# benfred/implicit

Hardware: AMD Instinct MI355X
Metric: ALS user+item updates/sec per iteration (factors=128); top-k recs/sec (higher is better)
Workload: dtype f32; 1 GPU; BASELINE configs[2]: last.fm-360K-shaped synthetic CSR, ALS CG cg_steps=3; users=358868, items=292385, nnz=17308340, factors=128, solver=cg, cg_steps=3

## Files before the change

### implicit_amd/csrc/als_cg_q.hip

```cpp
#include <type_traits>

#include "als_qtile.h"
#include "common.h"

namespace imp {

template <typename T>
void launch_team_fused(const imp_csr *C, int f, int width, int first, int count, T *X, const T *Y, const float *A0, int cg_steps,
                       const char *name);
template <typename T>
void launch_group_fused(const imp_csr *C, int f, int first, int count, T *X, const T *Y, const float *A0, int cg_steps, const char *name);
template <typename ST>
void launch_team_tile64(const imp_csr *C, int f, int width, int first, int count, ST *X, const ST *Y, const float *A0, int cg_steps,
                        const char *name);

template <int F, typename T> static void run_classes_q(const imp_csr *C, T *X, const T *Y, const float *A0, int cg_steps) {
  const int32_t *b = C->bin_start;
  constexpr bool kHalf = std::is_same<T, __half>::value;
  auto team = [&](int width32, int lo, int hi, const char *name) {
    if constexpr (kHalf) launch_team_tile64<T>(C, F, width32 / 2, lo, hi - lo, X, Y, A0, cg_steps, name);
    else launch_team_fused<T>(C, F, width32, lo, hi - lo, X, Y, A0, cg_steps, name);
  };
  team(16, b[1], b[2], "als_cg_team16_rows");
  team(8, b[2], b[3], "als_cg_team8_rows");
  team(4, b[3], b[4], "als_cg_team4_rows");
  team(2, b[4], b[5], "als_cg_team2_rows");
  if constexpr (F == 64) launch_team_fused<T>(C, F, 1, b[5], b[7] - b[5], X, Y, A0, cg_steps, "als_cg_short_rows");
  else launch_group_fused<T>(C, F, b[5], b[7] - b[5], X, Y, A0, cg_steps, "als_cg_short_rows");
}

template <typename T> void least_squares_cg_q(const imp_csr *C, T *X, const T *Y, const float *A0, int f, int cg_steps) {
  if (f == 128) run_classes_q<128, T>(C, X, Y, A0, cg_steps);
  else if (f == 64) run_classes_q<64, T>(C, X, Y, A0, cg_steps);
  else throw std::invalid_argument("least_squares_cg_q: f must be 64 or 128");
}
template void least_squares_cg_q<float>(const imp_csr *, float *, const float *, const float *, int, int);
template void least_squares_cg_q<__half>(const imp_csr *, __half *, const __half *, const float *, int, int);

}
```

### implicit_amd/csrc/als_cg_qf.hip

```cpp
#include <type_traits>

#include "als_qf_common.h"
#include "common.h"

namespace imp {

template <typename ST> struct Tile32 {
  typedef f32x2 elem;
  static constexpr int T = 32;
  static constexpr bool ROLL = std::is_same<ST, float>::value;
  static __device__ __forceinline__ void fetch(const int32_t *indices, const float *data, int lane, int k0, int end, int &col, float &c) {
    fetch_entries(indices, data, lane, k0, end, col, c);
  }
  template <int H> static __device__ __forceinline__ void gather(elem (&yq)[H], const ST *p) {
#pragma unroll
    for (int h = 0; h < H; h += 2) {
      const float4 v = load4(p + 32 * h);
      yq[h] = f32x2{v.x, v.y}, yq[h + 1] = f32x2{v.z, v.w};
    }
  }
  template <int H> static __device__ __forceinline__ float dot(const elem (&yq)[H], const f32x2 (&ve)[H]) {
    f32x2 s = yq[0] * ve[0];
#pragma unroll
    for (int h = 1; h < H; ++h) s = __builtin_elementwise_fma(yq[h], ve[h], s);
    return s.x + s.y;
  }
  template <int H> static __device__ __forceinline__ void axpy(const elem (&yq)[H], float w, f32x2 (&ae)[H]) {
    const f32x2 w2 = {w, w};
#pragma unroll
    for (int h = 0; h < H; ++h) ae[h] = __builtin_elementwise_fma(w2, yq[h], ae[h]);
  }
};

template <int F, int WPR, int BLOCK, typename ST>
__global__ __launch_bounds__(BLOCK, F == 64 ? 8 : 4) void als_cg_qfteam_kernel(const int32_t *__restrict__ order, int first, int count,
                                                                 const int32_t *__restrict__ indptr,
                                                                 const int32_t *__restrict__ indices,
                                                                 const float *__restrict__ data, ST *__restrict__ X,
                                                                 const ST *__restrict__ Y, const float *__restrict__ A0,
                                                                 int cg_steps) {
  team_rows<Tile32<ST>, F, WPR, BLOCK>(order, first, count, indptr, indices, data, X, Y, A0, cg_steps);
}

template <int F, int WPR, int BLOCK, typename T>
static void launch_qfteam(const imp_csr *C, int first, int count, T *X, const T *Y, const float *A0, int cg_steps,
                          const char *name) {
  if (count <= 0) return;
  constexpr int WAVES = BLOCK / 64, TEAMS = WAVES / WPR;
  size_t lds = team_lds_bytes<F, WPR, BLOCK, Tile32<T>::T>();
  auto kern = als_cg_qfteam_kernel<F, WPR, BLOCK, T>;
  IMP_CHECK_HIP(hipFuncSetAttribute(reinterpret_cast<const void *>(kern), hipFuncAttributeMaxDynamicSharedMemorySize, (int)lds));
  int per_cu = (int)std::max<size_t>(1, std::min<size_t>(2048 / BLOCK, (160 * 1024) / lds));
  constexpr int kBaseOversub = WPR <= 4 ? 4 : (WPR == 8 ? 2 : (F == 64 ? 2 : 1));
  int grid = std::min((count + TEAMS - 1) / TEAMS, ctx().num_cus * per_cu * std::max(kBaseOversub, ctx().oversub));
  IMP_PROF(name);
  kern<<<grid, BLOCK, lds, stream()>>>(C->order.data(), first, count, C->indptr.data(), C->indices.data(), C->data.data(), X, Y,
                                      A0, cg_steps);
  IMP_CHECK_HIP(hipGetLastError());
}

typedef float f32x4 __attribute__((ext_vector_type(4)));
template <int F> struct QFGroupCfg {
  static constexpr int LD = F + 8;
  static constexpr int LDB = F + 8;
  static constexpr int NT = F / 16;
  static constexpr int KH = 16 / NT;
  static constexpr int KB = (F / 16) / KH;
  static constexpr size_t lds_bytes = (size_t)3 * F * LDB * 2 + (size_t)3 * 16 * LDB * 2 +
                                      ((size_t)16 * LD + (size_t)KH * 16 * LD + 16 * 64) * sizeof(float);
};
typedef __bf16 bf16x8 __attribute__((ext_vector_type(8)));
typedef __bf16 bf16x2 __attribute__((ext_vector_type(2)));
__device__ __forceinline__ void split_bf16(float x, __bf16 &hi, __bf16 &mid, __bf16 &lo) {
  hi = (__bf16)x;
  const float r1 = x - (float)hi;
  mid = (__bf16)r1;
  lo = (__bf16)(r1 - (float)mid);
}

template <int F, bool FIRST, bool LAST, typename ST>
__device__ __forceinline__ void tile_pass(f32x2 (&y)[8][F / 32], float *cw, int cnt, const float *vrow, float (&acc)[F / 64], int lane,
                                          int cnt_nx, int &col_nx, float &c_nx, const ST *__restrict__ Y) {
  using Tile = Tile32<ST>;
  constexpr int FE = F / 16, H = FE / 2;
  if constexpr (LAST) {
    col_nx = opaque(col_nx);
    c_nx = __int_as_float(opaque(__float_as_int(c_nx)));
  }
  f32x2 ve[H], ae[H];
  const float *cwg;
  {
    const int ln = opaque(lane);
    const int g = ln >> 4, m = ln & 15;
#pragma unroll
    for (int e = 0; e < FE; e += 4) {
      const float4 t = *reinterpret_cast<const float4 *>(vrow + 16 * e + 4 * m);
      ve[e / 2] = f32x2{t.x, t.y}, ve[e / 2 + 1] = f32x2{t.z, t.w};
    }
    cwg = cw + g;
  }
#pragma unroll
  for (int h = 0; h < H; ++h) ae[h] = f32x2{0.f, 0.f};
  auto partial = [&](int q) { return Tile::template dot<H>(y[q], ve); };
  auto axpy = [&](int q, float w) { Tile::template axpy<H>(y[q], w, ae); };
  static_for<4>([&](auto Pc) {
    constexpr int P = decltype(Pc)::value;
    if (8 * P < cnt) {
      const float cm1_0 = cwg[8 * P], cm1_1 = cwg[8 * P + 4];
      float cp_0 = 0.f, cp_1 = 0.f;
      if constexpr (FIRST) cp_0 = cwg[32 + 8 * P], cp_1 = cwg[32 + 8 * P + 4];
      const float u = reduce_pair(partial(2 * P), partial(2 * P + 1));
      const float w0 = FIRST ? fmaf(-cm1_0, row_bcast_from<0>(u), cp_0) : cm1_0 * row_bcast_from<0>(u);
      const float w1 = FIRST ? fmaf(-cm1_1, row_bcast_from<8>(u), cp_1) : cm1_1 * row_bcast_from<8>(u);
      axpy(2 * P, w0);
      axpy(2 * P + 1, w1);
    }
    if constexpr (LAST) {
      if (8 * P < cnt_nx) gather_pair<Tile, F, P>(y, cw, col_nx, c_nx, cnt_nx, Y, lane);
    }
  });
  float aes[FE];
#pragma unroll
  for (int h = 0; h < H; ++h) aes[2 * h] = ae[h].x, aes[2 * h + 1] = ae[h].y;
  reduce_expanded<F>(aes, acc);
}

template <int F, typename ST>
__global__ __launch_bounds__(1024) void als_cg_qfgroup_kernel(const int32_t *__restrict__ order, int first, int count,
                                                              const int32_t *__restrict__ indptr,
                                                              const int32_t *__restrict__ indices,
                                                              const float *__restrict__ data, ST *__restrict__ X,
                                                              const ST *__restrict__ Y, const float *__restrict__ A0, int cg_steps) {
  using Cfg = QFGroupCfg<F>;
  constexpr int FC = F / 64, FE = F / 16, LD = Cfg::LD;
  constexpr bool ROLL = Tile32<ST>::ROLL;
  extern __shared__ __attribute__((aligned(16))) float smem[];
  constexpr int LDB = Cfg::LDB;
  __bf16 *A0b = reinterpret_cast<__bf16 *>(smem);
  __bf16 *Pb = A0b + (size_t)3 * F * LDB;
  float *Ps = reinterpret_cast<float *>(Pb + (size_t)3 * 16 * LDB);
  float *Outs = Ps + 16 * LD;
  float *cws = Outs + (size_t)Cfg::KH * 16 * LD;
  const int lane = threadIdx.x & 63;
  const int wave = __builtin_amdgcn_readfirstlane(threadIdx.x >> 6);
  for (int e = threadIdx.x; e < F * F; e += 1024) {
    int r = e / F, c = e - r * F;
    __bf16 h, m, l;
    split_bf16(A0[e], h, m, l);
    A0b[r * LDB + c] = h, A0b[(size_t)F * LDB + r * LDB + c] = m, A0b[(size_t)2 * F * LDB + r * LDB + c] = l;
  }
  __syncthreads();
  float *prow = Ps + (size_t)wave * LD;
  float *cw = cws + (size_t)wave * 64;
  const unsigned cf = (unsigned)QL<F>::cfactor(lane, 0);

  auto publish = [&](const float (&vec)[FC], bool valid) {
    if constexpr (FC == 2) *reinterpret_cast<float2 *>(prow + cf) = valid ? make_float2(vec[0], vec[1]) : make_float2(0.f, 0.f);
    else prow[cf] = valid ? vec[0] : 0.f;
    bf16x2 t[3];
#pragma unroll
    for (int c = 0; c < 2; ++c) {
      __bf16 h, m, l;
      split_bf16(valid ? vec[c] : 0.f, h, m, l);
      t[0][c] = h, t[1][c] = m, t[2][c] = l;
    }
#pragma unroll
    for (int k = 0; k < 3; ++k) *reinterpret_cast<bf16x2 *>(Pb + (size_t)k * 16 * LDB + (size_t)wave * LDB + cf) = t[k];
    __syncthreads();
  };
  auto product = [&]() {
    const int ti = wave % Cfg::NT, kh = wave / Cfg::NT;
    const int ln = opaque(lane);
    const int i = ln & 15, kq = ln >> 4;
    f32x4 acc = {0.f, 0.f, 0.f, 0.f};
    static_assert(Cfg::KB * 16 == 64, "three-term product: 64 k per wave");
#pragma unroll
    for (int b = 0; b < 2; ++b) {
      const int k0 = kh * 64 + 32 * b + 8 * kq;
      const __bf16 *ar = A0b + (size_t)(16 * ti + i) * LDB + k0, *pr = Pb + (size_t)i * LDB + k0;
      const bf16x8 ah = *reinterpret_cast<const bf16x8 *>(ar), am = *reinterpret_cast<const bf16x8 *>(ar + (size_t)F * LDB),
                   al = *reinterpret_cast<const bf16x8 *>(ar + (size_t)2 * F * LDB);
      const bf16x8 ph = *reinterpret_cast<const bf16x8 *>(pr), pm = *reinterpret_cast<const bf16x8 *>(pr + (size_t)16 * LDB),
                   pl = *reinterpret_cast<const bf16x8 *>(pr + (size_t)2 * 16 * LDB);
      acc = __builtin_amdgcn_mfma_f32_16x16x32_bf16(al, ph, acc, 0, 0, 0);
      acc = __builtin_amdgcn_mfma_f32_16x16x32_bf16(ah, pl, acc, 0, 0, 0);
      acc = __builtin_amdgcn_mfma_f32_16x16x32_bf16(am, pm, acc, 0, 0, 0);
      acc = __builtin_amdgcn_mfma_f32_16x16x32_bf16(am, ph, acc, 0, 0, 0);
      acc = __builtin_amdgcn_mfma_f32_16x16x32_bf16(ah, pm, acc, 0, 0, 0);
      acc = __builtin_amdgcn_mfma_f32_16x16x32_bf16(ah, ph, acc, 0, 0, 0);
    }
    *reinterpret_cast<float4 *>(Outs + (kh * 16 + i) * LD + 16 * ti + 4 * kq) = make_float4(acc[0], acc[1], acc[2], acc[3]);
  };
  auto collect = [&](float (&out)[FC]) {
#pragma unroll
    for (int c = 0; c < FC; ++c) out[c] = 0.f;
#pragma unroll
    for (int h = 0; h < Cfg::KH; ++h) {
      const float *o = Outs + (h * 16 + wave) * LD + cf;
      if constexpr (FC == 2) {
        const float2 t = *reinterpret_cast<const float2 *>(o);
        out[0] += t.x, out[1] += t.y;
      } else {
        out[0] += o[0];
      }
    }
  };
  const bool product_first = ((wave >> 2) & 1) == 0;

  const int groups = (count + 15) / 16, g_step = gridDim.x;
  auto row_id = [&](int g) { return order[first + min(g * 16 + wave, count - 1)]; };
  auto row_valid = [&](int g) { return g < groups && g * 16 + wave < count; };
  int id0 = row_id(blockIdx.x), id1 = row_id(blockIdx.x + g_step), id2 = row_id(blockIdx.x + 2 * g_step), id3 = row_id(blockIdx.x + 3 * g_step);
  int b0 = indptr[id0], e0 = indptr[id0 + 1], b1 = indptr[id1], e1 = indptr[id1 + 1], b2 = indptr[id2], e2 = indptr[id2 + 1];
  int ent_col, ent_cnt = row_valid(blockIdx.x) ? e0 - b0 : 0;
  float ent_c;
  fetch_entries(indices, data, opaque(lane), b0, max(e0, b0 + 1), ent_col, ent_c);
  bool tile_ready = false;
  int cnt = 0;
  f32x2 y[8][FE / 2];
  float x[FC];
  auto kill = [](float (&v)[FC]) {
#pragma unroll
    for (int cc = 0; cc < FC; ++cc) v[cc] = 0.f;
  };
  kill(x);
  for (int g = blockIdx.x; g < groups; g += g_step) {
    const bool valid = row_valid(g);
    ST *xrow = X + (size_t)id0 * F;
    if (!tile_ready) {
      cnt = ent_cnt;
      ent_col = opaque(ent_col);
      ent_c = __int_as_float(opaque(__float_as_int(ent_c)));
      static_for<4>([&](auto Pc) {
        constexpr int P = decltype(Pc)::value;
        if (8 * P < cnt) gather_pair<Tile32<ST>, F, P>(y, cw, ent_col, ent_c, cnt, Y, lane);
      });
      ent_cnt = row_valid(g + g_step) ? e1 - b1 : 0;
      fetch_entries(indices, data, opaque(lane), b1, max(e1, b1 + 1), ent_col, ent_c);
      load_compact<F>(xrow, opaque(lane), x);
    }
    float xc[FC], r[FC], p[FC], Ap[FC], sp[FC];
#pragma unroll
    for (int cc = 0; cc < FC; ++cc) xc[cc] = x[cc];
    publish(xc, valid);
    if (!product_first) tile_pass<F, true, false, ST>(y, cw, cnt, prow, sp, lane, 0, ent_col, ent_c, Y);
    product();
    if (product_first) tile_pass<F, true, false, ST>(y, cw, cnt, prow, sp, lane, 0, ent_col, ent_c, Y);
    __syncthreads();
    collect(Ap);
#pragma unroll
    for (int cc = 0; cc < FC; ++cc) p[cc] = r[cc] = sp[cc] - Ap[cc];
    float rsold = dot_compact<F>(r, r);
    bool active = valid && rsold >= 1e-20f;
    const bool store = active;
    for (int it = 0; it + 1 < cg_steps; ++it) {
      publish(p, active);
      if (active && !product_first) tile_pass<F, false, false, ST>(y, cw, cnt, prow, sp, lane, 0, ent_col, ent_c, Y);
      product();
      if (active && product_first) tile_pass<F, false, false, ST>(y, cw, cnt, prow, sp, lane, 0, ent_col, ent_c, Y);
      __syncthreads();
      collect(Ap);
      if (active) {
#pragma unroll
        for (int cc = 0; cc < FC; ++cc) Ap[cc] += sp[cc];
        const float alpha = rsold * __builtin_amdgcn_rcpf(dot_compact<F>(p, Ap));
#pragma unroll
        for (int cc = 0; cc < FC; ++cc) {
          xc[cc] = fmaf(alpha, p[cc], xc[cc]);
          r[cc] = fmaf(-alpha, Ap[cc], r[cc]);
        }
        const float rsnew = dot_compact<F>(r, r);
        if (rsnew < 1e-20f) {
          active = false;
        } else {
          const float beta = rsnew * __builtin_amdgcn_rcpf(rsold);
#pragma unroll
          for (int cc = 0; cc < FC; ++cc) p[cc] = fmaf(beta, p[cc], r[cc]);
          rsold = rsnew;
        }
      }
    }
    bool rolled = false;
    if (cg_steps > 0) {
      publish(p, active);
      auto last_tiles = [&]() {
        if constexpr (ROLL) tile_pass<F, false, true, ST>(y, cw, cnt, prow, sp, lane, ent_cnt, ent_col, ent_c, Y);
        else tile_pass<F, false, false, ST>(y, cw, cnt, prow, sp, lane, 0, ent_col, ent_c, Y);
      };
      if (active && !product_first) last_tiles();
      product();
      if (active && product_first) last_tiles();
      __syncthreads();
      collect(Ap);
      if (active) {
        if constexpr (ROLL) {
          cnt = ent_cnt;
          ent_cnt = row_valid(g + 2 * g_step) ? e2 - b2 : 0;
          fetch_entries(indices, data, opaque(lane), b2, max(e2, b2 + 1), ent_col, ent_c);
          load_compact<F>(X + (size_t)id1 * F, opaque(lane), x);
          rolled = true;
        } else {
          kill(x);
        }
#pragma unroll
        for (int cc = 0; cc < FC; ++cc) Ap[cc] += sp[cc];
        const float alpha = rsold * __builtin_amdgcn_rcpf(dot_compact<F>(p, Ap));
#pragma unroll
        for (int cc = 0; cc < FC; ++cc) xc[cc] = fmaf(alpha, p[cc], xc[cc]);
      } else {
        kill(x);
      }
    } else {
      kill(x);
    }
    if (store) store_compact<F>(xrow, opaque(lane), xc);
    tile_ready = rolled;
    id0 = id1, id1 = id2, id2 = id3, id3 = row_id(g + 4 * g_step);
    b0 = b1, e0 = e1, b1 = b2, e1 = e2, b2 = indptr[id2], e2 = indptr[id2 + 1];
  }
}

template <typename T>
static void launch_qfgroup(const imp_csr *C, int first, int count, T *X, const T *Y, const float *A0, int cg_steps, const char *name) {
  if (count <= 0) return;
  constexpr int F = 128;
  const size_t lds = QFGroupCfg<F>::lds_bytes;
  auto kern = als_cg_qfgroup_kernel<F, T>;
  IMP_CHECK_HIP(hipFuncSetAttribute(reinterpret_cast<const void *>(kern), hipFuncAttributeMaxDynamicSharedMemorySize, (int)lds));
  int grid = std::min((count + 15) / 16, ctx().num_cus * std::max(2, ctx().oversub));
  IMP_PROF(name);
  kern<<<grid, 1024, lds, stream()>>>(C->order.data(), first, count, C->indptr.data(), C->indices.data(), C->data.data(), X, Y, A0,
                                      cg_steps);
  IMP_CHECK_HIP(hipGetLastError());
}

template <typename T>
void launch_group_fused(const imp_csr *C, int f, int first, int count, T *X, const T *Y, const float *A0, int cg_steps, const char *name) {
  if (f == 128) launch_qfgroup<T>(C, first, count, X, Y, A0, cg_steps, name);
  else throw std::invalid_argument("launch_group_fused: f must be 128 (f = 64 short rows run on independent wavefronts)");
}
template void launch_group_fused<float>(const imp_csr *, int, int, int, float *, const float *, const float *, int, const char *);
template void launch_group_fused<__half>(const imp_csr *, int, int, int, __half *, const __half *, const float *, int, const char *);

template <typename T>
void launch_team_fused(const imp_csr *C, int f, int width, int first, int count, T *X, const T *Y, const float *A0, int cg_steps,
                       const char *name) {
  if constexpr (std::is_same<T, __half>::value) {
    if (f != 64 || width != 1) throw std::invalid_argument("launch_team_fused: float16 storage takes the f = 64 short rows only");
    launch_qfteam<64, 1, 512, T>(C, first, count, X, Y, A0, cg_steps, name);
  } else {
    auto run = [&](auto Fc) {
      constexpr int F = decltype(Fc)::value;
      switch (width) {
        case 16: launch_qfteam<F, 16, 1024, T>(C, first, count, X, Y, A0, cg_steps, name); break;
        case 8: launch_qfteam<F, 8, 512, T>(C, first, count, X, Y, A0, cg_steps, name); break;
        case 4: launch_qfteam<F, 4, 512, T>(C, first, count, X, Y, A0, cg_steps, name); break;
        case 2: launch_qfteam<F, 2, 512, T>(C, first, count, X, Y, A0, cg_steps, name); break;
        case 1:
          if constexpr (F == 64) launch_qfteam<F, 1, 512, T>(C, first, count, X, Y, A0, cg_steps, name);
          else throw std::invalid_argument("launch_team_fused: one wave per row needs f = 64");
          break;
        default: throw std::invalid_argument("launch_team_fused: team width");
      }
    };
    if (f == 128) run(idx_t<128>{});
    else if (f == 64) run(idx_t<64>{});
    else throw std::invalid_argument("launch_team_fused: f must be 64 or 128");
  }
}
template void launch_team_fused<float>(const imp_csr *, int, int, int, int, float *, const float *, const float *, int, const char *);
template void launch_team_fused<__half>(const imp_csr *, int, int, int, int, __half *, const __half *, const float *, int,
                                        const char *);

}
```

### implicit_amd/csrc/als_qf_common.h

```cpp
#ifndef IMPLICIT_AMD_CSRC_ALS_QF_COMMON_H_
#define IMPLICIT_AMD_CSRC_ALS_QF_COMMON_H_
#include <type_traits>
#include <utility>

#include "als_qtile.h"

namespace imp {

__device__ __forceinline__ int opaque(int v) {
  asm volatile("" : "+v"(v));
  return v;
}

typedef float f32x2 __attribute__((ext_vector_type(2)));

template <int I> using idx_t = std::integral_constant<int, I>;
template <int N, typename Fn, int... Is> __device__ __forceinline__ void static_for_impl(Fn &&fn, std::integer_sequence<int, Is...>) {
  (fn(idx_t<Is>{}), ...);
}
template <int N, typename Fn> __device__ __forceinline__ void static_for(Fn &&fn) {
  static_for_impl<N>(fn, std::make_integer_sequence<int, N>{});
}

template <int F, int NJ, int TICKS> struct DenseTicks {
  static constexpr int FE = F / 16, Q4 = FE / 4;
  static constexpr int EVERY = TICKS / NJ;
  static_assert(NJ >= 1 && NJ <= TICKS && TICKS % NJ == 0 && (NJ & (NJ - 1)) == 0, "steps per pass");
  float4 a[Q4];
  f32x2 vj2;
  template <int K> __device__ __forceinline__ void issue(const float *row, const float *vp) {
    if constexpr (K % EVERY == 0) {
      constexpr int s = K / EVERY;
      if constexpr (NJ == 1) vj2 = f32x2{vp[0], 0.f};
      else if constexpr (s % 2 == 0) vj2 = *reinterpret_cast<const f32x2 *>(vp + s);
#pragma unroll
      for (int e = 0; e < Q4; ++e) a[e] = *reinterpret_cast<const float4 *>(row + (size_t)s * F + 64 * e);
    }
  }
  template <int K> __device__ __forceinline__ void consume(f32x2 (&ae)[FE / 2]) {
    if constexpr (K % EVERY == 0) {
      constexpr int s = K / EVERY;
      const float vj = (s % 2 == 0) ? vj2.x : vj2.y;
      const f32x2 v2 = {vj, vj};
#pragma unroll
      for (int e = 0; e < Q4; ++e) {
        ae[2 * e] = __builtin_elementwise_fma(v2, f32x2{a[e].x, a[e].y}, ae[2 * e]);
        ae[2 * e + 1] = __builtin_elementwise_fma(v2, f32x2{a[e].z, a[e].w}, ae[2 * e + 1]);
      }
    }
  }
};

__device__ __forceinline__ float reduce_pair(float d0, float d1) {
  float u = d1 + dpp_mov<0x128>(d1);
  const float s0 = d0 + dpp_mov<0x128>(d0);
  u = __builtin_bit_cast(float, __builtin_amdgcn_update_dpp(__builtin_bit_cast(int, u), __builtin_bit_cast(int, s0), 0xE4, 0xF, 0x3,
                                                            false));
  u += dpp_mov<0x141>(u);
  u += dpp_mov<0xB1>(u);
  u += dpp_mov<0x4E>(u);
  return u;
}
template <int LANE> __device__ __forceinline__ float row_bcast_from(float v) {
  return dpp_mov<0x150 + LANE>(v);
}

enum : unsigned { kGo = 1u, kLast = 2u };

#ifndef IMP_TEAM_NAP_FIRST
#define IMP_TEAM_NAP_FIRST 6
#endif
#ifndef IMP_TEAM_NAP_NEXT
#define IMP_TEAM_NAP_NEXT 2
#endif
#ifndef IMP_TEAM_NAP_LEADER
#define IMP_TEAM_NAP_LEADER 1
#endif
#ifndef IMP_TEAM_LEADER_PRIO
#define IMP_TEAM_LEADER_PRIO 0
#endif


template <typename Tile, int F, int P, typename ST>
__device__ __forceinline__ void gather_pair(typename Tile::elem (&y)[Tile::T / 4][F / 32], float *cw, int col_reg, float c_reg, int cnt,
                                            const ST *__restrict__ Y, int lane) {
  lane = opaque(lane);
  if ((lane >> 3) == P) {
    const bool ok = lane < cnt;
    cw[lane] = ok ? fabsf(c_reg) - 1.f : 0.f;
    cw[Tile::T + lane] = ok ? fmaxf(c_reg, 0.f) : 0.f;
  }
  const int src = 4 * (lane >> 4);
#pragma unroll
  for (int q = 2 * P; q < 2 * P + 2; ++q) {
    const unsigned col = (unsigned)__builtin_amdgcn_ds_bpermute(src + 16 * q, col_reg);
    Tile::template gather<F / 32>(y[q], Y + (size_t)col * F + 4 * (lane & 15));
  }
}

template <typename Tile, int F, int NJ, bool FIRST, bool LAST, typename ST>
__device__ __forceinline__ void fused_pass(typename Tile::elem (&y)[Tile::T / 4][F / 32], float *cw, int cnt, const float *vt,
                                           int j_begin, const float *A0s, float (&acc)[F / 64], int lane, int cnt_nx, int &col_nx,
                                           float &c_nx, const ST *__restrict__ Y, const int32_t *__restrict__ indices,
                                           const float *__restrict__ data, int k0_nx2, int end_nx2) {
  constexpr int FE = F / 16, H = FE / 2, PAIRS = Tile::T / 8;
  if constexpr (LAST) {
    col_nx = opaque(col_nx);
    c_nx = __int_as_float(opaque(__float_as_int(c_nx)));
  }
  f32x2 ve[H], ae[H];
  const float *row, *vp, *cwg;
  {
    const int ln = opaque(lane);
    const int g = ln >> 4, m = ln & 15;
#pragma unroll
    for (int e = 0; e < FE; e += 4) {
      const float4 t = *reinterpret_cast<const float4 *>(vt + 16 * e + 4 * m);
      ve[e / 2] = f32x2{t.x, t.y}, ve[e / 2 + 1] = f32x2{t.z, t.w};
    }
    vp = vt + j_begin + g * NJ;
    row = A0s + (size_t)(j_begin + g * NJ) * F + 4 * m;
    cwg = cw + g;
  }
#pragma unroll
  for (int h = 0; h < H; ++h) ae[h] = f32x2{0.f, 0.f};
  DenseTicks<F, NJ, 4 * PAIRS> dt;
  auto partial = [&](int q) { return Tile::template dot<H>(y[q], ve); };
  auto axpy = [&](int q, float w) { Tile::template axpy<H>(y[q], w, ae); };
  static_for<PAIRS>([&](auto Pc) {
    constexpr int P = decltype(Pc)::value;
    if (8 * P < cnt) {
      dt.template issue<4 * P>(row, vp);
      const float cm1_0 = cwg[8 * P], cm1_1 = cwg[8 * P + 4];
      float cp_0 = 0.f, cp_1 = 0.f;
      if constexpr (FIRST) cp_0 = cwg[Tile::T + 8 * P], cp_1 = cwg[Tile::T + 8 * P + 4];
      __builtin_amdgcn_sched_barrier(0);
      const float d0 = partial(2 * P);
      __builtin_amdgcn_sched_barrier(0);
      dt.template consume<4 * P>(ae);
      dt.template issue<4 * P + 1>(row, vp);
      __builtin_amdgcn_sched_barrier(0);
      const float d1 = partial(2 * P + 1);
      const float u = reduce_pair(d0, d1);
      dt.template consume<4 * P + 1>(ae);
      const float w0 = FIRST ? fmaf(cm1_0, row_bcast_from<0>(u), -cp_0) : cm1_0 * row_bcast_from<0>(u);
      const float w1 = FIRST ? fmaf(cm1_1, row_bcast_from<8>(u), -cp_1) : cm1_1 * row_bcast_from<8>(u);
      __builtin_amdgcn_sched_barrier(0);
      dt.template issue<4 * P + 2>(row, vp);
      __builtin_amdgcn_sched_barrier(0);
      axpy(2 * P, w0);
      __builtin_amdgcn_sched_barrier(0);
      dt.template consume<4 * P + 2>(ae);
      dt.template issue<4 * P + 3>(row, vp);
      __builtin_amdgcn_sched_barrier(0);
      axpy(2 * P + 1, w1);
      __builtin_amdgcn_sched_barrier(0);
      dt.template consume<4 * P + 3>(ae);
    } else {
      asm volatile("" ::: "memory");
      static_for<4>([&](auto Kc) {
        constexpr int K = 4 * P + decltype(Kc)::value;
        dt.template issue<K>(row, vp);
        __builtin_amdgcn_sched_barrier(0);
        dt.template consume<K>(ae);
      });
    }
    if constexpr (LAST) {
      if (8 * P < cnt_nx) gather_pair<Tile, F, P>(y, cw, col_nx, c_nx, cnt_nx, Y, lane);
    }
    __builtin_amdgcn_sched_barrier(0);
  });
  float aes[FE];
#pragma unroll
  for (int h = 0; h < H; ++h) aes[2 * h] = ae[h].x, aes[2 * h + 1] = ae[h].y;
  reduce_expanded<F>(aes, acc);
  if constexpr (LAST) {
    Tile::fetch(indices, data, opaque(lane), k0_nx2, end_nx2, col_nx, c_nx);
  }
}

template <int F, int WPR, int BLOCK, int T> constexpr size_t team_lds_bytes() {
  constexpr size_t WAVES = BLOCK / 64, TEAMS = WAVES / WPR;
  return ((size_t)F * F + WAVES * F + TEAMS * F + 2 * T * WAVES + 4 * TEAMS) * sizeof(float);
}

template <typename Tile, int F, int WPR, int BLOCK, typename ST>
__device__ __forceinline__ void team_rows(const int32_t *__restrict__ order, int first, int count, const int32_t *__restrict__ indptr,
                                          const int32_t *__restrict__ indices, const float *__restrict__ data, ST *__restrict__ X,
                                          const ST *__restrict__ Y, const float *__restrict__ A0, int cg_steps) {
  constexpr int FC = F / 64, FE = F / 16, T = Tile::T, WAVES = BLOCK / 64, TEAMS = WAVES / WPR, NJ = F / WPR / 4;
  static_assert(WPR <= WAVES && (F / WPR) % 4 == 0, "team width");
  extern __shared__ __attribute__((aligned(16))) float smem[];
  float *A0s = smem;
  float *parts = A0s + (size_t)F * F;
  float *vts = parts + (size_t)WAVES * F;
  float *cws = vts + (size_t)TEAMS * F;
  unsigned *ctl = reinterpret_cast<unsigned *>(cws + (size_t)WAVES * 2 * T);
  const int lane = threadIdx.x & 63;
  const int wave = __builtin_amdgcn_readfirstlane(threadIdx.x >> 6);
  const int team = wave / WPR, sub = wave % WPR;
  const bool leader = sub == 0;
  for (int e = threadIdx.x; e < F * F; e += BLOCK) A0s[e] = A0[e];
  if (threadIdx.x < 4 * TEAMS) ctl[threadIdx.x] = 0u;
  __syncthreads();
  const int j_begin = F * sub / WPR;
  float *vt = vts + (size_t)team * F;
  float *cw = cws + (size_t)wave * 2 * T;
  unsigned *arrivals = ctl + 4 * team, *generation = arrivals + 1, *words = arrivals + 2;

  unsigned gen = 0, pub = 0, arr_target = 0;
  auto lds_off = [](const void *ptr) { return (unsigned)(size_t)ptr; };
  const unsigned arrivals_off = lds_off(arrivals), generation_off = lds_off(generation), words_off = lds_off(words);
  const unsigned cf4 = 4u * (unsigned)QL<F>::cfactor(lane, 0);
  auto publish = [&](unsigned w) {
    ++pub;
    if (lane == 0)
      asm volatile("ds_write_b32 %0, %1\n\tds_add_u32 %2, %3" ::"v"(words_off + 4u * (pub & 1u)), "v"(w), "v"(generation_off), "v"(1u)
                   : "memory");
    if constexpr (IMP_TEAM_LEADER_PRIO > 0) __builtin_amdgcn_s_setprio(0);
  };
  auto poll = [&](unsigned off) {
    typedef __attribute__((address_space(3))) volatile unsigned lds_word;
    return (unsigned)__builtin_amdgcn_readfirstlane(*(lds_word *)(size_t)off);
  };
  auto await_operand = [&]() -> unsigned {
    ++gen;
    if constexpr (WPR > 1) {
      if (poll(generation_off) < gen) {
        __builtin_amdgcn_s_sleep(IMP_TEAM_NAP_FIRST);
        while (poll(generation_off) < gen) __builtin_amdgcn_s_sleep(IMP_TEAM_NAP_NEXT);
      }
    }
    return poll(words_off + 4u * (gen & 1u));
  };
  auto arrive = [&](const float (&acc)[FC]) {
    float *slot = reinterpret_cast<float *>(reinterpret_cast<char *>(parts + (size_t)wave * F) + cf4);
    if constexpr (FC == 2) *reinterpret_cast<float2 *>(slot) = make_float2(acc[0], acc[1]);
    else slot[0] = acc[0];
    if constexpr (WPR > 1) {
      if (lane == 0) asm volatile("ds_add_u32 %0, %1" ::"v"(arrivals_off), "v"(1u) : "memory");
    }
  };
  auto collect = [&](float (&acc)[FC]) {
    arr_target += WPR;
    if constexpr (WPR > 1) {
      while (poll(arrivals_off) < arr_target) __builtin_amdgcn_s_sleep(IMP_TEAM_NAP_LEADER);
    }
    if constexpr (IMP_TEAM_LEADER_PRIO > 0) __builtin_amdgcn_s_setprio(IMP_TEAM_LEADER_PRIO);
    const float *slot = reinterpret_cast<const float *>(reinterpret_cast<const char *>(parts + (size_t)(team * WPR) * F) + cf4);
#pragma unroll
    for (int c = 0; c < FC; ++c) acc[c] = 0.f;
#pragma unroll
    for (int w = 0; w < WPR; ++w) {
      if constexpr (FC == 2) {
        const float2 t = *reinterpret_cast<const float2 *>(slot + (size_t)w * F);
        acc[0] += t.x, acc[1] += t.y;
      } else {
        acc[0] += slot[(size_t)w * F];
      }
    }
  };
  auto operand_slot = [&]() { return reinterpret_cast<float *>(reinterpret_cast<char *>(vt) + cf4); };
  auto put_operand = [&](const float (&v)[FC]) {
    float *slot = operand_slot();
    if constexpr (FC == 2) *reinterpret_cast<float2 *>(slot) = make_float2(v[0], v[1]);
    else slot[0] = v[0];
  };
  auto get_operand = [&](float (&v)[FC]) {
    const float *slot = operand_slot();
    if constexpr (FC == 2) {
      const float2 t = *reinterpret_cast<const float2 *>(slot);
      v[0] = t.x, v[1] = t.y;
    } else {
      v[0] = slot[0];
    }
  };

  auto row_id = [&](int i) { return order[first + min(i, count - 1)]; };
  const int i_step = gridDim.x * TEAMS, i_first = blockIdx.x * TEAMS + team;
  auto slice = [&](int rb, int re, int &k0, int &cnt) {
    const int chunk = min(T, (((re - rb) + WPR - 1) / WPR + 3) & ~3);
    k0 = min(rb + chunk * sub, re);
    cnt = min(chunk, re - k0);
  };
  int id0 = row_id(i_first), id1 = row_id(i_first + i_step), id2 = row_id(i_first + 2 * i_step), id3 = row_id(i_first + 3 * i_step);
  int b0 = indptr[id0], e0 = indptr[id0 + 1], b1 = indptr[id1], e1 = indptr[id1 + 1], b2 = indptr[id2], e2 = indptr[id2 + 1];
  int ent_col, ent_cnt, k0;
  float ent_c;
  slice(b0, e0, k0, ent_cnt);
  Tile::fetch(indices, data, opaque(lane), k0, max(k0 + ent_cnt, b0 + 1), ent_col, ent_c);
  auto kill = [](float (&v)[FC]) {
#pragma unroll
    for (int cc = 0; cc < FC; ++cc) v[cc] = 0.f;
  };
  bool tile_ready = false;
  int cnt = 0;
  typename Tile::elem y[T / 4][FE / 2];
  float x[FC];
  kill(x);
  for (int i = i_first; i < count; i += i_step) {
    ST *xrow = X + (size_t)id0 * F;
    if (!tile_ready) {
      cnt = ent_cnt;
      ent_col = opaque(ent_col);
      ent_c = __int_as_float(opaque(__float_as_int(ent_c)));
      static_for<T / 8>([&](auto Pc) {
        constexpr int P = decltype(Pc)::value;
        if (8 * P < cnt) gather_pair<Tile, F, P>(y, cw, ent_col, ent_c, cnt, Y, lane);
      });
      slice(b1, e1, k0, ent_cnt);
      Tile::fetch(indices, data, opaque(lane), k0, max(k0 + ent_cnt, b1 + 1), ent_col, ent_c);
      if (leader) load_compact<F>(xrow, opaque(lane), x);
      else kill(x);
    }
    float xc[FC], r[FC], p[FC], Ap[FC], rsold = 0.f;
#pragma unroll
    for (int cc = 0; cc < FC; ++cc) xc[cc] = r[cc] = 0.f;
    bool store = false;
    if (leader) {
      put_operand(x);
#pragma unroll
      for (int cc = 0; cc < FC; ++cc) xc[cc] = x[cc];
      publish(kGo);
    }
    unsigned w = await_operand();
    {
      float acc[FC];
      fused_pass<Tile, F, NJ, true, false>(y, cw, cnt, vt, j_begin, A0s, acc, lane, 0, ent_col, ent_c, Y, nullptr, nullptr, 0, 0);
      arrive(acc);
    }
    if (leader) {
      collect(r);
#pragma unroll
      for (int cc = 0; cc < FC; ++cc) r[cc] = -r[cc], p[cc] = r[cc];
      rsold = dot_compact<F>(r, r);
      store = rsold >= 1e-20f;
      if (store && cg_steps > 0) {
        put_operand(p);
        publish(kGo | (cg_steps == 1 ? kLast : 0u));
      } else {
        publish(0u);
      }
    }
    w = await_operand();
    for (int it = 0; (w & (kGo | kLast)) == kGo; ++it) {
      float acc[FC];
      fused_pass<Tile, F, NJ, false, false>(y, cw, cnt, vt, j_begin, A0s, acc, lane, 0, ent_col, ent_c, Y, nullptr, nullptr, 0, 0);
      arrive(acc);
      if (leader) {
        collect(Ap);
        get_operand(p);
        const float alpha = rsold * __builtin_amdgcn_rcpf(dot_compact<F>(p, Ap));
#pragma unroll
        for (int cc = 0; cc < FC; ++cc) {
          xc[cc] = fmaf(alpha, p[cc], xc[cc]);
          r[cc] = fmaf(-alpha, Ap[cc], r[cc]);
        }
        const float rsnew = dot_compact<F>(r, r);
        if (rsnew < 1e-20f) {
          publish(0u);
        } else {
          const float beta = rsnew * __builtin_amdgcn_rcpf(rsold);
#pragma unroll
          for (int cc = 0; cc < FC; ++cc) p[cc] = fmaf(beta, p[cc], r[cc]);
          rsold = rsnew;
          put_operand(p);
          publish(kGo | (it + 2 >= cg_steps ? kLast : 0u));
        }
      }
      w = await_operand();
    }
    const bool rolled = Tile::ROLL && (w & kGo) != 0u;
    if (w & kGo) {
      float acc[FC];
      if constexpr (Tile::ROLL) {
        int k2, cnt2;
        slice(b2, e2, k2, cnt2);
        if (i + i_step >= count) ent_cnt = 0;
        fused_pass<Tile, F, NJ, false, true>(y, cw, cnt, vt, j_begin, A0s, acc, lane, ent_cnt, ent_col, ent_c, Y, indices, data, k2,
                                             max(k2 + cnt2, b2 + 1));
        cnt = ent_cnt;
        ent_cnt = cnt2;
        if (leader) load_compact<F>(X + (size_t)id1 * F, opaque(lane), x);
        else kill(x);
      } else {
        kill(x);
        fused_pass<Tile, F, NJ, false, false>(y, cw, cnt, vt, j_begin, A0s, acc, lane, 0, ent_col, ent_c, Y, nullptr, nullptr, 0, 0);
      }
      arrive(acc);
      if (leader) {
        collect(Ap);
        get_operand(p);
        const float alpha = rsold * __builtin_amdgcn_rcpf(dot_compact<F>(p, Ap));
#pragma unroll
        for (int cc = 0; cc < FC; ++cc) xc[cc] = fmaf(alpha, p[cc], xc[cc]);
        publish(0u);
      }
      (void)await_operand();
    } else {
      kill(x);
    }
    if (leader && store) store_compact<F>(xrow, opaque(lane), xc);
    tile_ready = rolled;
    id0 = id1, id1 = id2, id2 = id3, id3 = row_id(i + 4 * i_step);
    b0 = b1, e0 = e1, b1 = b2, e1 = e2, b2 = indptr[id2], e2 = indptr[id2 + 1];
  }
}

}
#endif
```

Baseline: 162.5 million updates/s.

## Fuse team8/team4/team2 CG launches into one persistent multi-class kernel

Replaces three separate kernel launches, one per row-length class (team widths 8, 4, 2), with a single persistent kernel that processes each class in turn. The A0 matrix is loaded into LDS once per block, and separate control-word slots are kept for each class. The intent is to remove per-launch overhead, repeated A0 staging and the tail idle time between dependent launches. In exchange the combined kernel sizes its LDS for the narrowest width, which may lower occupancy, and the oversubscription defaults for the team kernels change.

```diff
diff --git a/implicit_amd/csrc/als_cg_q.hip b/implicit_amd/csrc/als_cg_q.hip
--- a/implicit_amd/csrc/als_cg_q.hip
+++ b/implicit_amd/csrc/als_cg_q.hip
@@ -8,6 +8,8 @@
 template <typename T>
 void launch_team_fused(const imp_csr *C, int f, int width, int first, int count, T *X, const T *Y, const float *A0, int cg_steps,
                        const char *name);
+template <typename T>
+void launch_team_classes_fused(const imp_csr *C, int f, T *X, const T *Y, const float *A0, int cg_steps, const char *name);
 template <typename T>
 void launch_group_fused(const imp_csr *C, int f, int first, int count, T *X, const T *Y, const float *A0, int cg_steps, const char *name);
 template <typename ST>
@@ -22,9 +24,13 @@
     else launch_team_fused<T>(C, F, width32, lo, hi - lo, X, Y, A0, cg_steps, name);
   };
   team(16, b[1], b[2], "als_cg_team16_rows");
-  team(8, b[2], b[3], "als_cg_team8_rows");
-  team(4, b[3], b[4], "als_cg_team4_rows");
-  team(2, b[4], b[5], "als_cg_team2_rows");
+  if constexpr (kHalf) {
+    team(8, b[2], b[3], "als_cg_team8_rows");
+    team(4, b[3], b[4], "als_cg_team4_rows");
+    team(2, b[4], b[5], "als_cg_team2_rows");
+  } else {
+    launch_team_classes_fused<T>(C, F, X, Y, A0, cg_steps, "als_cg_team8_rows");
+  }
   if constexpr (F == 64) launch_team_fused<T>(C, F, 1, b[5], b[7] - b[5], X, Y, A0, cg_steps, "als_cg_short_rows");
   else launch_group_fused<T>(C, F, b[5], b[7] - b[5], X, Y, A0, cg_steps, "als_cg_short_rows");
 }
diff --git a/implicit_amd/csrc/als_cg_qf.hip b/implicit_amd/csrc/als_cg_qf.hip
--- a/implicit_amd/csrc/als_cg_qf.hip
+++ b/implicit_amd/csrc/als_cg_qf.hip
@@ -51,13 +51,60 @@
   auto kern = als_cg_qfteam_kernel<F, WPR, BLOCK, T>;
   IMP_CHECK_HIP(hipFuncSetAttribute(reinterpret_cast<const void *>(kern), hipFuncAttributeMaxDynamicSharedMemorySize, (int)lds));
   int per_cu = (int)std::max<size_t>(1, std::min<size_t>(2048 / BLOCK, (160 * 1024) / lds));
-  constexpr int kBaseOversub = WPR <= 4 ? 4 : (WPR == 8 ? 2 : (F == 64 ? 2 : 1));
+  constexpr int kBaseOversub = WPR == 1 ? 4 : (F == 64 ? 2 : 1);
   int grid = std::min((count + TEAMS - 1) / TEAMS, ctx().num_cus * per_cu * std::max(kBaseOversub, ctx().oversub));
   IMP_PROF(name);
   kern<<<grid, BLOCK, lds, stream()>>>(C->order.data(), first, count, C->indptr.data(), C->indices.data(), C->data.data(), X, Y,
                                       A0, cg_steps);
   IMP_CHECK_HIP(hipGetLastError());
 }
+
+template <int F, typename ST>
+__global__ __launch_bounds__(512, F == 64 ? 8 : 4) void als_cg_qfteam_kernel_classes(const int32_t *__restrict__ order,
+                                                                                     const TeamClassRanges rg,
+                                                                                     const int32_t *__restrict__ indptr,
+                                                                                     const int32_t *__restrict__ indices,
+                                                                                     const float *__restrict__ data, ST *__restrict__ X,
+                                                                                     const ST *__restrict__ Y, const float *__restrict__ A0,
+                                                                                     int cg_steps) {
+  team_rows_classes<Tile32<ST>, F, 8, 4, 2, 512>(order, rg, indptr, indices, data, X, Y, A0, cg_steps);
+}
+
+#ifndef IMP_TEAM_CLASSES_OVERSUB
+#define IMP_TEAM_CLASSES_OVERSUB 4
+#endif
+
+template <int F, typename T>
+static void launch_qfteam_classes(const imp_csr *C, const TeamClassRanges &rg, T *X, const T *Y, const float *A0, int cg_steps,
+                                  const char *name) {
+  constexpr int BLOCK = 512, WAVES = BLOCK / 64;
+  constexpr int kWidth[3] = {8, 4, 2};
+  int want = 0;
+  for (int k = 0; k < 3; ++k) {
+    const int teams = WAVES / kWidth[k];
+    want = std::max(want, (std::max(rg.count[k], 0) + teams - 1) / teams);
+  }
+  if (want <= 0) return;
+  using L = TeamLds<F, BLOCK, Tile32<T>::T, 2, 3>;
+  const size_t lds = L::bytes;
+  auto kern = als_cg_qfteam_kernel_classes<F, T>;
+  IMP_CHECK_HIP(hipFuncSetAttribute(reinterpret_cast<const void *>(kern), hipFuncAttributeMaxDynamicSharedMemorySize, (int)lds));
+  const int per_cu = (int)std::max<size_t>(1, std::min<size_t>(2048 / BLOCK, (160 * 1024) / lds));
+  const int grid = std::min(want, ctx().num_cus * per_cu * std::max(IMP_TEAM_CLASSES_OVERSUB, ctx().oversub));
+  IMP_PROF(name);
+  kern<<<grid, BLOCK, lds, stream()>>>(C->order.data(), rg, C->indptr.data(), C->indices.data(), C->data.data(), X, Y, A0, cg_steps);
+  IMP_CHECK_HIP(hipGetLastError());
+}
+
+template <typename T> void launch_team_classes_fused(const imp_csr *C, int f, T *X, const T *Y, const float *A0, int cg_steps, const char *name) {
+  const int32_t *b = C->bin_start;
+  TeamClassRanges rg;
+  for (int k = 0; k < 3; ++k) rg.first[k] = b[2 + k], rg.count[k] = b[3 + k] - b[2 + k];
+  if (f == 128) launch_qfteam_classes<128, T>(C, rg, X, Y, A0, cg_steps, name);
+  else if (f == 64) launch_qfteam_classes<64, T>(C, rg, X, Y, A0, cg_steps, name);
+  else throw std::invalid_argument("launch_team_classes_fused: f must be 64 or 128");
+}
+template void launch_team_classes_fused<float>(const imp_csr *, int, float *, const float *, const float *, int, const char *);
 
 typedef float f32x4 __attribute__((ext_vector_type(4)));
 template <int F> struct QFGroupCfg {
@@ -353,9 +400,6 @@
       constexpr int F = decltype(Fc)::value;
       switch (width) {
         case 16: launch_qfteam<F, 16, 1024, T>(C, first, count, X, Y, A0, cg_steps, name); break;
-        case 8: launch_qfteam<F, 8, 512, T>(C, first, count, X, Y, A0, cg_steps, name); break;
-        case 4: launch_qfteam<F, 4, 512, T>(C, first, count, X, Y, A0, cg_steps, name); break;
-        case 2: launch_qfteam<F, 2, 512, T>(C, first, count, X, Y, A0, cg_steps, name); break;
         case 1:
           if constexpr (F == 64) launch_qfteam<F, 1, 512, T>(C, first, count, X, Y, A0, cg_steps, name);
           else throw std::invalid_argument("launch_team_fused: one wave per row needs f = 64");
diff --git a/implicit_amd/csrc/als_qf_common.h b/implicit_amd/csrc/als_qf_common.h
--- a/implicit_amd/csrc/als_qf_common.h
+++ b/implicit_amd/csrc/als_qf_common.h
@@ -179,32 +179,40 @@
   }
 }
 
-template <int F, int WPR, int BLOCK, int T> constexpr size_t team_lds_bytes() {
-  constexpr size_t WAVES = BLOCK / 64, TEAMS = WAVES / WPR;
-  return ((size_t)F * F + WAVES * F + TEAMS * F + 2 * T * WAVES + 4 * TEAMS) * sizeof(float);
-}
-
-template <typename Tile, int F, int WPR, int BLOCK, typename ST>
-__device__ __forceinline__ void team_rows(const int32_t *__restrict__ order, int first, int count, const int32_t *__restrict__ indptr,
-                                          const int32_t *__restrict__ indices, const float *__restrict__ data, ST *__restrict__ X,
-                                          const ST *__restrict__ Y, const float *__restrict__ A0, int cg_steps) {
+template <int F, int BLOCK, int T, int WMIN, int NW> struct TeamLds {
+  static constexpr int WAVES = BLOCK / 64, SLOTS = WAVES / WMIN;
+  static constexpr size_t parts = (size_t)F * F, vts = parts + (size_t)WAVES * F, cws = vts + (size_t)SLOTS * F,
+                          ctl = cws + (size_t)WAVES * 2 * T, ctl_words = (size_t)NW * SLOTS * 4;
+  static constexpr size_t bytes = (ctl + ctl_words) * sizeof(float);
+};
+template <int F, int WPR, int BLOCK, int T> constexpr size_t team_lds_bytes() { return TeamLds<F, BLOCK, T, WPR, 1>::bytes; }
+
+template <typename L, int F, int BLOCK> __device__ __forceinline__ void team_prologue(const float *__restrict__ A0) {
+  extern __shared__ __attribute__((aligned(16))) float smem[];
+  unsigned *ctl = reinterpret_cast<unsigned *>(smem + L::ctl);
+  for (int e = threadIdx.x; e < F * F; e += BLOCK) smem[e] = A0[e];
+  static_assert(L::ctl_words <= BLOCK, "control words");
+  if (threadIdx.x < L::ctl_words) ctl[threadIdx.x] = 0u;
+  __syncthreads();
+}
+
+template <typename Tile, int F, int WPR, int BLOCK, typename L, int KW, typename ST>
+__device__ __forceinline__ void team_class_rows(const int lane, const int wave, const int32_t *__restrict__ order, int first, int count,
+                                                const int32_t *__restrict__ indptr, const int32_t *__restrict__ indices,
+                                                const float *__restrict__ data, ST *__restrict__ X, const ST *__restrict__ Y,
+                                                int cg_steps) {
   constexpr int FC = F / 64, FE = F / 16, T = Tile::T, WAVES = BLOCK / 64, TEAMS = WAVES / WPR, NJ = F / WPR / 4;
-  static_assert(WPR <= WAVES && (F / WPR) % 4 == 0, "team width");
+  static_assert(WPR <= WAVES && (F / WPR) % 4 == 0 && TEAMS <= L::SLOTS && L::SLOTS % TEAMS == 0, "team width");
   extern __shared__ __attribute__((aligned(16))) float smem[];
   float *A0s = smem;
-  float *parts = A0s + (size_t)F * F;
-  float *vts = parts + (size_t)WAVES * F;
-  float *cws = vts + (size_t)TEAMS * F;
-  unsigned *ctl = reinterpret_cast<unsigned *>(cws + (size_t)WAVES * 2 * T);
-  const int lane = threadIdx.x & 63;
-  const int wave = __builtin_amdgcn_readfirstlane(threadIdx.x >> 6);
+  float *parts = smem + L::parts;
+  float *vts = smem + L::vts;
+  float *cws = smem + L::cws;
+  unsigned *ctl = reinterpret_cast<unsigned *>(smem + L::ctl) + KW * L::SLOTS * 4;
   const int team = wave / WPR, sub = wave % WPR;
   const bool leader = sub == 0;
-  for (int e = threadIdx.x; e < F * F; e += BLOCK) A0s[e] = A0[e];
-  if (threadIdx.x < 4 * TEAMS) ctl[threadIdx.x] = 0u;
-  __syncthreads();
   const int j_begin = F * sub / WPR;
-  float *vt = vts + (size_t)team * F;
+  float *vt = vts + (size_t)(team * (L::SLOTS / TEAMS)) * F;
   float *cw = cws + (size_t)wave * 2 * T;
   unsigned *arrivals = ctl + 4 * team, *generation = arrivals + 1, *words = arrivals + 2;
 
@@ -407,5 +415,34 @@
   }
 }
 
+template <typename Tile, int F, int WPR, int BLOCK, typename ST>
+__device__ __forceinline__ void team_rows(const int32_t *__restrict__ order, int first, int count, const int32_t *__restrict__ indptr,
+                                          const int32_t *__restrict__ indices, const float *__restrict__ data, ST *__restrict__ X,
+                                          const ST *__restrict__ Y, const float *__restrict__ A0, int cg_steps) {
+  using L = TeamLds<F, BLOCK, Tile::T, WPR, 1>;
+  const int lane = threadIdx.x & 63;
+  const int wave = __builtin_amdgcn_readfirstlane(threadIdx.x >> 6);
+  team_prologue<L, F, BLOCK>(A0);
+  team_class_rows<Tile, F, WPR, BLOCK, L, 0>(lane, wave, order, first, count, indptr, indices, data, X, Y, cg_steps);
+}
+
+struct TeamClassRanges {
+  int first[3], count[3];
+};
+template <typename Tile, int F, int W0, int W1, int W2, int BLOCK, typename ST>
+__device__ __forceinline__ void team_rows_classes(const int32_t *__restrict__ order, const TeamClassRanges rg,
+                                                  const int32_t *__restrict__ indptr, const int32_t *__restrict__ indices,
+                                                  const float *__restrict__ data, ST *__restrict__ X, const ST *__restrict__ Y,
+                                                  const float *__restrict__ A0, int cg_steps) {
+  static_assert(W0 > W1 && W1 > W2, "widest team first");
+  using L = TeamLds<F, BLOCK, Tile::T, W2, 3>;
+  auto lane_id = []() { return opaque((int)__builtin_amdgcn_mbcnt_hi(~0u, __builtin_amdgcn_mbcnt_lo(~0u, 0u))); };
+  const int wave = __builtin_amdgcn_readfirstlane(threadIdx.x >> 6);
+  team_prologue<L, F, BLOCK>(A0);
+  if (rg.count[0] > 0) team_class_rows<Tile, F, W0, BLOCK, L, 0>(lane_id(), wave, order, rg.first[0], rg.count[0], indptr, indices, data, X, Y, cg_steps);
+  if (rg.count[1] > 0) team_class_rows<Tile, F, W1, BLOCK, L, 1>(lane_id(), wave, order, rg.first[1], rg.count[1], indptr, indices, data, X, Y, cg_steps);
+  if (rg.count[2] > 0) team_class_rows<Tile, F, W2, BLOCK, L, 2>(lane_id(), wave, order, rg.first[2], rg.count[2], indptr, indices, data, X, Y, cg_steps);
+}
+
 }
 #endif
```

New measurement: 163.8 million updates/s, median of 6. Within noise of the previous version (+0.8%).
